# irconde/SSL4POLYP

Hardware: AMD Instinct MI355X
Metric: training-step images/sec/node, ViT-B/16 224^2 (cls fine-tune) (higher is better)
Workload: dtype bf16; 1 GPU; ViT-B/16 classification fine-tune, bs=64/GPU, 224^2, AdamW, random init, finetune mode full (finetune.py:49-91); global_batch=64, parallelism=dp1, launch=eager, lr_schedule=constant

## Files before the change

ssl4polyp_amd/csrc/pm_layernorm.hip:

```cpp
#include "pm_common.h"

namespace {

constexpr int kMaxD = 1280;

template <typename TOut, int NV>
__global__ __launch_bounds__(256) void ln_fwd_kernel(const float* __restrict__ x, long ldx, const float* __restrict__ gamma,
                                                     const float* __restrict__ beta, TOut* __restrict__ y,
                                                     float* __restrict__ mean_out, float* __restrict__ rstd_out, int M,
                                                     int D, float eps) {
  constexpr int kMaxVec = NV;
  const int lane = threadIdx.x & 63;
  const int wave = threadIdx.x >> 6;
  const int nvec = D >> 2;
  for (long row = (long)blockIdx.x * 4 + wave; row < M; row += (long)gridDim.x * 4) {
    const float* xr = x + row * ldx;
    f32x4 v[kMaxVec];
    float s = 0.f;
#pragma unroll
    for (int i = 0; i < kMaxVec; ++i) {
      const int c = lane + 64 * i;
      if (c < nvec) {
        v[i] = *reinterpret_cast<const f32x4*>(xr + 4 * c);
        s += (v[i][0] + v[i][1]) + (v[i][2] + v[i][3]);
// ... 31 lines not shown
      }
    }
  }
}

template <typename TDy, typename TAct, int NV>
__global__ __launch_bounds__(256) void ln_bwd_kernel(const TDy* __restrict__ dy, const float* __restrict__ x, long ldx,
                                                     const float* __restrict__ gamma, const float* __restrict__ mean,
                                                     const float* __restrict__ rstd, const float* __restrict__ dres,
                                                     long lddres, float* __restrict__ dx, long lddx,
                                                     TAct* __restrict__ dx_act, float* __restrict__ dgamma,
                                                     float* __restrict__ dbeta, float* __restrict__ dcolsum,
                                                     float* __restrict__ partials, int M, int D) {
  __shared__ float red[3][4][256 + 4];
  constexpr int kMaxVec = NV;
  const int lane = threadIdx.x & 63;
  const int wave = threadIdx.x >> 6;
  const int nvec = D >> 2;
  f32x4 g[kMaxVec];
  f32x4 acc_g[kMaxVec], acc_b[kMaxVec], acc_c[kMaxVec];
#pragma unroll
  for (int i = 0; i < kMaxVec; ++i) {
    const int c = lane + 64 * i;
    const f32x4 z = {0.f, 0.f, 0.f, 0.f};
    g[i] = (c < nvec) ? *reinterpret_cast<const f32x4*>(gamma + 4 * c) : z;
    acc_g[i] = z;
    acc_b[i] = z;
    acc_c[i] = z;
  }
  const float invD = 1.0f / (float)D;
  const long stride = (long)gridDim.x * 4;
  for (long row0 = (long)blockIdx.x * 4 + wave; row0 < M; row0 += 2 * stride) {
    long rows[2] = {row0, row0 + stride};
    const bool valid[2] = {true, rows[1] < M};
    if (!valid[1]) rows[1] = row0;
    float mu[2], rs[2], s1[2] = {0.f, 0.f}, s2[2] = {0.f, 0.f};
    f32x4 xh[2][kMaxVec], dv[2][kMaxVec], dr[2][kMaxVec];
#pragma unroll
    for (int u = 0; u < 2; ++u) {
      mu[u] = mean[rows[u]];
      rs[u] = rstd[rows[u]];
#pragma unroll
      for (int i = 0; i < kMaxVec; ++i) {
        const int c = lane + 64 * i;
        if (c < nvec) {
          xh[u][i] = *reinterpret_cast<const f32x4*>(x + rows[u] * ldx + 4 * c);
          dv[u][i] = load4<TDy>(dy + rows[u] * (long)D + 4 * c);
          if (dres) dr[u][i] = *reinterpret_cast<const f32x4*>(dres + rows[u] * lddres + 4 * c);
        }
      }
    }
#pragma unroll
    for (int u = 0; u < 2; ++u) {
      const float live = valid[u] ? 1.0f : 0.0f;
#pragma unroll
      for (int i = 0; i < kMaxVec; ++i) {
        const int c = lane + 64 * i;
        if (c < nvec) {
#pragma unroll
          for (int e = 0; e < 4; ++e) {
            xh[u][i][e] = (xh[u][i][e] - mu[u]) * rs[u];
            const float gg = dv[u][i][e] * g[i][e];
            s1[u] += gg;
            s2[u] += gg * xh[u][i][e];
            acc_g[i][e] += live * dv[u][i][e] * xh[u][i][e];
            acc_b[i][e] += live * dv[u][i][e];
          }
        }
      }
    }
    float c1[2], c2[2];
#pragma unroll
    for (int u = 0; u < 2; ++u) {
      c1[u] = s1[u];
      c2[u] = s2[u];
    }
#pragma unroll
    for (int o = 32; o > 0; o >>= 1) {
      c1[0] += __shfl_xor(c1[0], o, 64);
      c1[1] += __shfl_xor(c1[1], o, 64);
      c2[0] += __shfl_xor(c2[0], o, 64);
      c2[1] += __shfl_xor(c2[1], o, 64);
    }
#pragma unroll
    for (int u = 0; u < 2; ++u) {
      if (!valid[u]) continue;
      const float k1 = c1[u] * invD, k2 = c2[u] * invD;
#pragma unroll
      for (int i = 0; i < kMaxVec; ++i) {
        const int c = lane + 64 * i;
        if (c < nvec) {
          f32x4 o;
#pragma unroll
          for (int e = 0; e < 4; ++e) o[e] = rs[u] * (dv[u][i][e] * g[i][e] - k1 - xh[u][i][e] * k2);
          if (dres) o += dr[u][i];
          *reinterpret_cast<f32x4*>(dx + rows[u] * lddx + 4 * c) = o;
          if (dx_act) store4<TAct>(dx_act + rows[u] * (long)D + 4 * c, o);
#pragma unroll
          for (int e = 0; e < 4; ++e) acc_c[i][e] += o[e];
        }
      }
    }
  }
#pragma unroll
  for (int i = 0; i < kMaxVec; ++i) {
    const int c = lane + 64 * i;
    __syncthreads();
#pragma unroll
    for (int e = 0; e < 4; ++e) {
      red[0][wave][lane * 4 + e] = acc_g[i][e];
      red[1][wave][lane * 4 + e] = acc_b[i][e];
      red[2][wave][lane * 4 + e] = acc_c[i][e];
    }
    __syncthreads();
    if (wave < 3 && c < nvec) {
      float* dst = wave == 0 ? dgamma : (wave == 1 ? dbeta : dcolsum);
      if (dst) {
        f32x4 t;
#pragma unroll
        for (int e = 0; e < 4; ++e)
          t[e] = (red[wave][0][lane * 4 + e] + red[wave][1][lane * 4 + e]) +
                 (red[wave][2][lane * 4 + e] + red[wave][3][lane * 4 + e]);
        if (partials) {
          *reinterpret_cast<f32x4*>(partials + ((long)blockIdx.x * 3 + wave) * D + 4 * c) = t;
        } else {
#pragma unroll
          for (int e = 0; e < 4; ++e) atomicAdd(dst + 4 * c + e, t[e]);
        }
      }
    }
  }
}

__global__ __launch_bounds__(1024) void ln_bwd_reduce_kernel(const float* __restrict__ partials, float* dgamma, float* dbeta,
                                                             float* dcolsum, int nblocks, int D) {
  __shared__ float red[16][64];
  const int lane = threadIdx.x & 63, rg = threadIdx.x >> 6;
  const int d = blockIdx.x * 64 + lane;
  const int v = blockIdx.y;
  float* dst = v == 0 ? dgamma : (v == 1 ? dbeta : dcolsum);
  if (!dst) return;
  float s0 = 0.f;
  if (d < D) s0 = strided_sum<16>(partials + (long)v * D + d, 3L * D, rg, 16, nblocks);
  red[rg][lane] = s0;
  __syncthreads();
  if (rg == 0 && d < D) {
    float t = 0.f;
#pragma unroll
    for (int g = 0; g < 16; ++g) t += red[g][lane];
    dst[d] += t;
  }
}

inline int ln_grid(int M) {
  int g = (M + 3) / 4;
  return g < 1 ? 1 : (g > 1024 ? 1024 : g);
}

}

extern "C" int pm_layernorm_fwd(const float* x, long ldx, const float* gamma, const float* beta, void* y, int out_dtype,
                                float* mean, float* rstd, int M, int D, float eps, void* stream) {
  if (!x || !gamma || !beta || !y || !mean || !rstd) return PM_EINVAL;
  if (M <= 0 || D <= 0 || D > kMaxD || (D & 3) || (ldx & 3)) return PM_ESHAPE;
  const int grid = (M + 3) / 4 > 4096 ? 4096 : (M + 3) / 4;
#define PM_LN_FWD(TO, NV) \
  hipLaunchKernelGGL((ln_fwd_kernel<TO, NV>), dim3(grid), dim3(256), 0, pm_stream(stream), x, ldx, gamma, beta, (TO*)y, mean, rstd, M, D, eps)
  PM_DISPATCH_ACT(out_dtype, T, {
    if (D <= 1024) PM_LN_FWD(T, 4); else PM_LN_FWD(T, 5);
  });
#undef PM_LN_FWD
  return pm_check_launch();
}

extern "C" int pm_layernorm_bwd(const void* dy, int dy_dtype, const float* x, long ldx, const float* gamma,
                                const float* mean, const float* rstd, const float* dres, long lddres, float* dx,
                                long lddx, void* dx_act, int act_dtype, float* dgamma, float* dbeta, float* dcolsum,
                                int M, int D, void* workspace, size_t ws_bytes, void* stream) {
  if (!dy || !x || !gamma || !mean || !rstd || !dx) return PM_EINVAL;
  if (M <= 0 || D <= 0 || D > kMaxD || (D & 3) || (ldx & 3) || (lddx & 3) || (dres && (lddres & 3))) return PM_ESHAPE;
  if (dx_act && act_dtype != dy_dtype) return PM_EINVAL;
  int grid = (M + 3) / 4;
  float* partials = nullptr;
  const bool want_sums = dgamma || dbeta || dcolsum;
  if (want_sums && workspace && ws_bytes >= (size_t)64 * 3 * D * sizeof(float)) {
    int cap = (int)(ws_bytes / ((size_t)3 * D * sizeof(float)));
    if (cap > 1024) cap = 1024;
    if (grid > cap) grid = cap;
    partials = reinterpret_cast<float*>(workspace);
  } else if (grid > 256) {
    grid = 256;
  }
  if (grid < 1) grid = 1;
  hipStream_t s = pm_stream(stream);
  const int nv = (D + 255) / 256;
#define PM_LN_BWD(TD, NV)                                                                                               \
  hipLaunchKernelGGL((ln_bwd_kernel<TD, TD, NV>), dim3(grid), dim3(256), 0, s, (const TD*)dy, x, ldx, gamma, mean, rstd, \
                     dres, lddres, dx, lddx, (TD*)dx_act, dgamma, dbeta, dcolsum, partials, M, D)
  PM_DISPATCH_ACT(dy_dtype, T, {
    if (nv == 1) PM_LN_BWD(T, 1); else if (nv == 2) PM_LN_BWD(T, 2); else if (nv == 3) PM_LN_BWD(T, 3);
    else if (nv == 4) PM_LN_BWD(T, 4); else PM_LN_BWD(T, 5);
  });
#undef PM_LN_BWD
  if (partials)
    hipLaunchKernelGGL(ln_bwd_reduce_kernel, dim3((D + 63) / 64, 3), dim3(1024), 0, s, partials, dgamma, dbeta, dcolsum, grid, D);
  return pm_check_launch();
}
```

ssl4polyp_amd/csrc/pm_attention.hip:

```cpp
#include "pm_common.h"
#include <stdlib.h>

namespace {

template <int DH> constexpr int kTileUnroll = DH == 32 ? 2 : 1;

template <int RB> __device__ __forceinline__ int swz(int row) {
  if constexpr (RB == 64) return (row >> 2) & 3;
  else if constexpr (RB == 128) return (((row >> 1) & 1) << 2) | ((row >> 2) & 3);
  else if constexpr (RB == 384) return row & 7;
  else return row & 15;
}

template <typename T, int DH> constexpr int row_bytes() {
  return DH == 80 ? (sizeof(T) == 2 ? 256 : 384) : DH * (int)sizeof(T);
}

template <typename T, int DH>
__device__ __forceinline__ void load_image(char* img, const T* __restrict__ src, long ld, int rows_valid,
                                           int rows_total, int tid, int nthreads) {
  constexpr int RB = row_bytes<T, DH>();
  constexpr int CPV = DH * sizeof(T) / 16;
  constexpr int CPF = ((DH + 31) / 32) * 32 * sizeof(T) / 16;
  constexpr int EPC = 16 / sizeof(T);
  for (int id = tid; id < rows_total * CPF; id += nthreads) {
    const int row = id / CPF, c = id % CPF;
    u32x4 v = {0u, 0u, 0u, 0u};
    if (row < rows_valid && c < CPV) v = *reinterpret_cast<const u32x4*>(src + (long)row * ld + c * EPC);
    *reinterpret_cast<u32x4*>(img + row * RB + 16 * (c ^ swz<RB>(row))) = v;
  }
}

template <typename T, int DH>
__device__ __forceinline__ Frag16 frag_rows(const char* img, int rb, int kk, int lane) {
  constexpr int RB = row_bytes<T, DH>();
  const int row = rb + (lane & 31);
  const int c = 2 * kk + (lane >> 5);
  Frag16 f;
  f.u = *reinterpret_cast<const u32x4*>(img + row * RB + 16 * (c ^ swz<RB>(row)));
  return f;
}

template <typename T>
__device__ __forceinline__ Frag16 frag_global(const T* __restrict__ rowptr, bool valid, int kk, int lane) {
  constexpr int EPC = 16 / sizeof(T);
  Frag16 f;
  f.u = (u32x4){0u, 0u, 0u, 0u};
  if (valid) f.u = *reinterpret_cast<const u32x4*>(rowptr + (2 * kk + (lane >> 5)) * EPC);
  return f;
}

template <typename T, int DH>
__device__ __forceinline__ f32x16 mma_imgT_acc(const char* PM_LDS_IMAGE img, int rb, int d0, const f32x16& x, f32x16 acc, int lane) {
  constexpr int RB = row_bytes<T, DH>();
  if constexpr (sizeof(T) == 2) {
    const int g = lane >> 4, i = lane & 15, q = i >> 2, p = i & 3, hh = g >> 1;
    const int col = d0 + 16 * (g & 1) + 4 * p;
    const int c = col >> 3, sub = 8 * (p & 1);
    using lds_s4 = __attribute__((address_space(3))) short4v;
#pragma unroll
    for (int s = 0; s < 2; ++s) {
      Frag16 a, b;
      const int r0 = rb + 16 * s + 4 * hh + q;
      const int r1 = r0 + 8;
      const short4v lo = __builtin_amdgcn_ds_read_tr16_b64_v4i16((lds_s4*)(img + r0 * RB + 16 * (c ^ swz<RB>(r0)) + sub));
      const short4v hi = __builtin_amdgcn_ds_read_tr16_b64_v4i16((lds_s4*)(img + r1 * RB + 16 * (c ^ swz<RB>(r1)) + sub));
      a.u[0] = ((unsigned)(unsigned short)lo[0]) | (((unsigned)(unsigned short)lo[1]) << 16);
      a.u[1] = ((unsigned)(unsigned short)lo[2]) | (((unsigned)(unsigned short)lo[3]) << 16);
      a.u[2] = ((unsigned)(unsigned short)hi[0]) | (((unsigned)(unsigned short)hi[1]) << 16);
      a.u[3] = ((unsigned)(unsigned short)hi[2]) | (((unsigned)(unsigned short)hi[3]) << 16);
#pragma unroll
      for (int j = 0; j < 8; ++j) frag_set<T>(b, j, x[8 * s + j]);
      acc = mfma16B<T>(a, b, acc);
    }
  } else {
    const int hh = lane >> 5;
    const int col = d0 + (lane & 31);
#pragma unroll
    for (int r = 0; r < 16; ++r) {
      const int row = rb + acc_row(r, hh);
      const float a = *reinterpret_cast<const float*>(img + row * RB + 16 * ((col >> 2) ^ swz<RB>(row)) + 4 * (col & 3));
      acc = __builtin_amdgcn_mfma_f32_32x32x2f32(a, x[r], acc, 0, 0, 0);
    }
  }
  return acc;
}

__device__ __forceinline__ f32x16 zero16() {
  f32x16 z;
#pragma unroll
  for (int r = 0; r < 16; ++r) z[r] = 0.f;
  return z;
}

template <typename T>
__device__ __forceinline__ void store_tile_T(T* __restrict__ rowptr, bool valid, const f32x16& acc, float scale, int lane,
                                             int ncols = 32) {
  if (!valid) return;
  const int hh = lane >> 5;
#pragma unroll
  for (int g = 0; g < 4; ++g) {
    f32x4 v = {acc[4 * g] * scale, acc[4 * g + 1] * scale, acc[4 * g + 2] * scale, acc[4 * g + 3] * scale};
    if (8 * g + 4 * hh < ncols) store4<T>(rowptr + 8 * g + 4 * hh, v);
  }
}
template <int DH> __device__ __forceinline__ constexpr int tile_cols(int dt) { return DH - 32 * dt < 32 ? DH - 32 * dt : 32; }

constexpr float kLog2e = 1.4426950408889634f;

struct QkvLayout {
  long ld, which_stride, head_stride, batch_stride;
};
inline QkvLayout qkv_layout(int B, int N, int H, int DH, bool head_major) {
  if (head_major) return QkvLayout{(long)DH, (long)B * H * N * DH, (long)N * DH, (long)H * N * DH};
  return QkvLayout{3L * H * DH, (long)H * DH, (long)DH, (long)N * 3L * H * DH};
}
inline bool attn_head_major() {
  static const bool v = [] { const char* e = getenv("PM_ATTN_HEADMAJOR"); return e && e[0] == '1'; }();
  return v;
}

template <int DH> __device__ __forceinline__ int problem_of_block(int bid, int nprob, int H) {
  if constexpr (DH == 32) {
#ifndef PM_ATTN_NO_PAIR_MAP
    if ((nprob & 15) == 0 && (H & 1) == 0) {
      const int xcd = bid & 7, j = bid >> 3;
      return (((j >> 1) << 3) + xcd) * 2 + (j & 1);
    }
#endif
  }
  return bid;
}

template <int NT> struct Waves { static constexpr int value = NT; };

template <typename T, int DH, int NT> constexpr int chunk_tiles() {
  constexpr int per_tile = 2 * 32 * row_bytes<T, DH>() + 2 * 32 * (int)sizeof(float);
  if (NT * per_tile <= 150 * 1024) return NT;
  return (80 * 1024) / per_tile;
}

template <typename T, int DH, int NT, int CT>
__global__ __launch_bounds__(Waves<NT>::value * 64) void attn_fwd_kernel(const T* __restrict__ qkv, T* __restrict__ out,
                                                                        float* __restrict__ lse, int N, int H,
                                                                        float scale) {
  constexpr int RB = row_bytes<T, DH>();
  constexpr int KS = DH * sizeof(T) / 32;
  constexpr int DT = (DH + 31) / 32;
  constexpr int NW = Waves<NT>::value;
  static_assert(NW == NT, "one wave per query tile: its softmax state stays in registers across key chunks");
  extern __shared__ __attribute__((aligned(16))) char smem[];
  char* imgK = smem;
  char* imgV = smem + CT * 32 * RB;
  const int tid = threadIdx.x, lane = tid & 63, wave = tid >> 6, hh = lane >> 5;
  const int prob = problem_of_block<DH>(blockIdx.x, gridDim.x, H);
  const int b = prob / H, h = prob % H;
  const long ld = 3L * H * DH;
  const T* base = qkv + (long)b * N * ld + h * DH;
  const float c = scale * kLog2e;
  const int q = wave * 32 + (lane & 31);
  const bool qv = q < N;
  Frag16 fq[KS];
  f32x16 o[DT];
#pragma unroll
  for (int dt = 0; dt < DT; ++dt) o[dt] = zero16();
  float m = -INFINITY, l = 0.f;
  for (int c0 = 0; c0 < NT; c0 += CT) {
    if (c0) __syncthreads();
    load_image<T, DH>(imgK, base + H * DH + (long)c0 * 32 * ld, ld, N - c0 * 32, CT * 32, tid, NW * 64);
    load_image<T, DH>(imgV, base + 2 * H * DH + (long)c0 * 32 * ld, ld, N - c0 * 32, CT * 32, tid, NW * 64);
    __syncthreads();
    if (c0 == 0) {
#pragma unroll
      for (int kk = 0; kk < KS; ++kk) fq[kk] = frag_global<T>(base + (long)q * ld, qv, kk, lane);
    }
    const int cend = c0 + CT < NT ? c0 + CT : NT;
#pragma unroll 1
    for (int kt = c0; kt < cend; ++kt) {
      const int rb = (kt - c0) * 32;
      f32x16 s = zero16();
#pragma unroll
      for (int kk = 0; kk < KS; ++kk) s = mfma16B<T>(frag_rows<T, DH>(imgK, rb, kk, lane), fq[kk], s);
      float tm = -INFINITY;
      if (kt * 32 + 32 > N) {
#pragma unroll
        for (int r = 0; r < 16; ++r) {
          const int key = kt * 32 + acc_row(r, hh);
          s[r] = key < N ? s[r] : -INFINITY;
        }
      }
#pragma unroll
      for (int r = 0; r < 16; ++r) tm = fmaxf(tm, s[r]);
      tm = fmaxf(tm, __shfl_xor(tm, 32, 64));
      const float mn = fmaxf(m, tm);
      const float alpha = __builtin_amdgcn_exp2f((m - mn) * c);
      const float mnc = mn * c;
      float ts = 0.f;
#pragma unroll
      for (int r = 0; r < 16; ++r) {
        s[r] = __builtin_amdgcn_exp2f(s[r] * c - mnc);
        ts += s[r];
      }
      l = l * alpha + ts;
      const bool moved = __builtin_amdgcn_ballot_w64(mn != m) != 0;
      m = mn;
#pragma unroll
      for (int dt = 0; dt < DT; ++dt) {
        if (moved) {
#pragma unroll
          for (int r = 0; r < 16; ++r) o[dt][r] *= alpha;
        }
        o[dt] = mma_imgT_acc<T, DH>(imgV, rb, dt * 32, s, o[dt], lane);
      }
    }
  }
  l += __shfl_xor(l, 32, 64);
  if (qv && hh == 0) lse[((long)b * H + h) * N + q] = m * scale + __logf(l);
  const float inv = 1.0f / l;
  T* orow = out + ((long)b * N + q) * H * DH + h * DH;
#pragma unroll
  for (int dt = 0; dt < DT; ++dt) store_tile_T<T>(orow + dt * 32, qv, o[dt], inv, lane, tile_cols<DH>(dt));
}

// ... 316 lines not shown
  const int b = prob / H, h = prob % H;
  const long ld = 3L * H * DH, ldo = (long)H * DH;
  const T* base = qkv + (long)b * lay.batch_stride + (long)h * lay.head_stride;
  const T* dobase = dout + (long)b * N * ldo + h * DH;
#pragma unroll
  for (int i = 0; i < (PCS + NT - 1) / NT; ++i) {
    const int p = wave + NT * i;
    if (p < PCS) {
      dma_rows<RB>(imgQ, base, lay.ld, N, p, lane);
      dma_rows<RB>(imgK, base + lay.which_stride, lay.ld, N, p, lane);
      dma_rows<RB>(imgV, base + 2 * lay.which_stride, lay.ld, N, p, lane);
      dma_rows<RB>(imgDO, dobase, ldo, N, p, lane);
    }
  }
  const int q = wave * 32 + (lane & 31);
  const bool qv = q < N;
  const long sidx = ((long)b * H + h) * N;
  Frag16 fo[KS];
  {
    const T* orow = out + ((long)b * N + (qv ? q : N - 1)) * ldo + h * DH;
#pragma unroll
    for (int kk = 0; kk < KS; ++kk) fo[kk].u = *reinterpret_cast<const u32x4*>(orow + (2 * kk + hh) * 8);
  }
  for (int i = tid; i < NT * 32; i += NT * 64) sl2[i] = i < N ? lse[sidx + i] * kLog2e : 0.f;
  asm volatile("s_waitcnt vmcnt(0)" ::: "memory");
  __syncthreads();
  {
    const int pad0 = N, npad = NT * 32 - N;
    for (int i = tid; i < npad * CPR; i += NT * 64) {
      const int off = (pad0 + i / CPR) * RB + 16 * (i % CPR);
      const u32x4 z = {0u, 0u, 0u, 0u};
      *reinterpret_cast<u32x4*>(imgQ + off) = z;
      *reinterpret_cast<u32x4*>(imgK + off) = z;
      *reinterpret_cast<u32x4*>(imgV + off) = z;
      *reinterpret_cast<u32x4*>(imgDO + off) = z;
    }
  }
  __syncthreads();
  const float c = scale * kLog2e;
  Frag16 fq[KS], fdo[KS];
  float dl = 0.f;
#pragma unroll
  for (int kk = 0; kk < KS; ++kk) {
    fq[kk] = frag_rows<T, DH>(imgQ, wave * 32, kk, lane);
    fdo[kk] = frag_rows<T, DH>(imgDO, wave * 32, kk, lane);
#pragma unroll
    for (int e = 0; e < 8; ++e) dl += frag_get<T>(fdo[kk], e) * frag_get<T>(fo[kk], e);
  }
  dl += __shfl_xor(dl, 32, 64);
  if (!qv) dl = 0.f;
  if (hh == 0) sdl[q] = dl * scale;
  {
    const float l2 = sl2[q];
    const float dls = dl * scale;
    f32x16 dq[DT];
#pragma unroll
    for (int dt = 0; dt < DT; ++dt) dq[dt] = zero16();
#pragma unroll kTileUnroll<DH>
    for (int kt = 0; kt < ((dbg & 1) ? 0 : NT); ++kt) {
      f32x16 s = zero16(), dp = zero16();
#pragma unroll
      for (int kk = 0; kk < KS; ++kk) {
        s = mfma16B<T>(frag_rows<T, DH>(imgK, kt * 32, kk, lane), fq[kk], s);
        dp = mfma16B<T>(frag_rows<T, DH>(imgV, kt * 32, kk, lane), fdo[kk], dp);
      }
#pragma unroll
      for (int r = 0; r < 16; ++r) s[r] = __builtin_amdgcn_exp2f(fminf(s[r] * c - l2, 0.f)) * (dp[r] * scale - dls);
#pragma unroll
      for (int dt = 0; dt < DT; ++dt) dq[dt] = mma_imgT_acc<T, DH>(imgK, kt * 32, dt * 32, s, dq[dt], lane);
    }
    T* dqrow = dqkv + ((long)b * N + q) * ld + h * DH;
#pragma unroll
    for (int dt = 0; dt < DT; ++dt) store_tile_T<T>(dqrow + dt * 32, qv, dq[dt], 1.0f, lane);
  }
  __syncthreads();
  {
    const int key = q;
    const bool kv = qv;
    Frag16 fk[KS], fv[KS];
#pragma unroll
    for (int kk = 0; kk < KS; ++kk) {
      fk[kk] = frag_rows<T, DH>(imgK, wave * 32, kk, lane);
      fv[kk] = frag_rows<T, DH>(imgV, wave * 32, kk, lane);
    }
    f32x16 dk[DT], dv[DT];
#pragma unroll
    for (int dt = 0; dt < DT; ++dt) {
      dk[dt] = zero16();
      dv[dt] = zero16();
    }
#pragma unroll kTileUnroll<DH>
    for (int qt = 0; qt < ((dbg & 2) ? 0 : NT); ++qt) {
      f32x16 s = zero16(), dp = zero16();
#pragma unroll
      for (int kk = 0; kk < KS; ++kk) {
        s = mfma16B<T>(frag_rows<T, DH>(imgQ, qt * 32, kk, lane), fk[kk], s);
        dp = mfma16B<T>(frag_rows<T, DH>(imgDO, qt * 32, kk, lane), fv[kk], dp);
      }
#pragma unroll
      for (int g = 0; g < 4; ++g) {
        const int qq = qt * 32 + 8 * g + 4 * hh;
        const f32x4 l4 = *reinterpret_cast<const f32x4*>(sl2 + qq);
        const f32x4 d4 = *reinterpret_cast<const f32x4*>(sdl + qq);
#pragma unroll
        for (int e = 0; e < 4; ++e) {
          const int r = 4 * g + e;
          const float pr = __builtin_amdgcn_exp2f(fminf(s[r] * c - l4[e], 0.f));
          s[r] = pr;
          dp[r] = pr * (dp[r] * scale - d4[e]);
        }
      }
#pragma unroll
      for (int dt = 0; dt < DT; ++dt) {
        dv[dt] = mma_imgT_acc<T, DH>(imgDO, qt * 32, dt * 32, s, dv[dt], lane);
        dk[dt] = mma_imgT_acc<T, DH>(imgQ, qt * 32, dt * 32, dp, dk[dt], lane);
      }
    }
    T* drow = dqkv + ((long)b * N + key) * ld + h * DH;
#pragma unroll
    for (int dt = 0; dt < DT; ++dt) {
      store_tile_T<T>(drow + H * DH + dt * 32, kv, dk[dt], 1.0f, lane);
      store_tile_T<T>(drow + 2 * H * DH + dt * 32, kv, dv[dt], 1.0f, lane);
    }
  }
}

template <typename T, int DH, int NT>
int launch_bwd_fused(const void* qkv, const void* out, const void* dout, const float* lse, void* dqkv, int B, int N, int H,
                     hipStream_t s) {
  const size_t lds = 4 * NT * 32 * DH * 2 + 2 * NT * 32 * sizeof(float);
  const float scale = 1.0f / sqrtf((float)DH);
  auto kern = attn_bwd_fused_kernel<T, DH, NT>;
  PM_ALLOW_LDS(kern, lds);
#ifdef PM_ATTN_DEBUG
  static const int dbg = [] { const char* e = getenv("PM_ATTN_BWD_SKIP"); return e ? atoi(e) : 0; }();
  hipLaunchKernelGGL(kern, dim3(B * H), dim3(NT * 64), lds, s, (const T*)qkv, (const T*)out, (const T*)dout, lse,
                     (T*)dqkv, N, H, scale, qkv_layout(B, N, H, DH, attn_head_major()), dbg);
#else
  hipLaunchKernelGGL(kern, dim3(B * H), dim3(NT * 64), lds, s, (const T*)qkv, (const T*)out, (const T*)dout, lse,
                     (T*)dqkv, N, H, scale, qkv_layout(B, N, H, DH, attn_head_major()));
#endif
  return pm_check_launch();
}

template <typename T, int DH>
int dispatch_bwd_fused(int nt, const void* qkv, const void* out, const void* dout, const float* lse, void* dqkv, int B, int N,
                       int H, hipStream_t s) {
  if (nt <= 1) return launch_bwd_fused<T, DH, 1>(qkv, out, dout, lse, dqkv, B, N, H, s);
  if (nt <= 2) return launch_bwd_fused<T, DH, 2>(qkv, out, dout, lse, dqkv, B, N, H, s);
  if (nt <= 7) return launch_bwd_fused<T, DH, 7>(qkv, out, dout, lse, dqkv, B, N, H, s);
  return launch_bwd_fused<T, DH, 9>(qkv, out, dout, lse, dqkv, B, N, H, s);
}

template <typename T, int DH, int NT>
int launch_bwd(const void* qkv, const void* out, const void* dout, const float* lse, float* delta, void* dqkv, int B,
               int N, int H, hipStream_t s) {
  constexpr int NW = Waves<NT>::value;
  constexpr int CT = chunk_tiles<T, DH, NT>();
  const size_t lds = 2 * CT * 32 * row_bytes<T, DH>();
  const size_t lds_kv = lds + 2 * CT * 32 * sizeof(float);
  const float scale = 1.0f / sqrtf((float)DH);
  auto kq = attn_bwd_q_kernel<T, DH, NT, CT>;
  auto kkv = attn_bwd_kv_kernel<T, DH, NT, CT>;
  PM_ALLOW_LDS(kq, lds);
  PM_ALLOW_LDS(kkv, lds_kv);
  hipLaunchKernelGGL(kq, dim3(B * H), dim3(NW * 64), lds, s, (const T*)qkv, (const T*)out, (const T*)dout, lse, delta,
                     (T*)dqkv, N, H, scale);
  hipLaunchKernelGGL(kkv, dim3(B * H), dim3(NW * 64), lds_kv, s, (const T*)qkv, (const T*)dout, lse,
                     (const float*)delta, (T*)dqkv, N, H, scale);
  return pm_check_launch();
}

template <typename T, int DH>
int dispatch_fwd(int nt, const void* qkv, void* out, float* lse, int B, int N, int H, hipStream_t s) {
  if constexpr (DH == 80) {
    if (nt <= 3) return launch_fwd<T, DH, 3>(qkv, out, lse, B, N, H, s);
    return launch_fwd<T, DH, 9>(qkv, out, lse, B, N, H, s);
  } else {
    if (nt <= 1) return launch_fwd<T, DH, 1>(qkv, out, lse, B, N, H, s);
    if (nt <= 2) return launch_fwd<T, DH, 2>(qkv, out, lse, B, N, H, s);
    if (nt <= 7) return launch_fwd<T, DH, 7>(qkv, out, lse, B, N, H, s);
    return launch_fwd<T, DH, 9>(qkv, out, lse, B, N, H, s);
  }
}
template <typename T, int DH>
int dispatch_bwd(int nt, const void* qkv, const void* out, const void* dout, const float* lse, float* delta, void* dqkv,
                 int B, int N, int H, hipStream_t s) {
  if constexpr (DH == 80) {
    if (nt <= 3) return launch_bwd<T, DH, 3>(qkv, out, dout, lse, delta, dqkv, B, N, H, s);
    return launch_bwd<T, DH, 9>(qkv, out, dout, lse, delta, dqkv, B, N, H, s);
  } else {
    if (nt <= 1) return launch_bwd<T, DH, 1>(qkv, out, dout, lse, delta, dqkv, B, N, H, s);
    if (nt <= 2) return launch_bwd<T, DH, 2>(qkv, out, dout, lse, delta, dqkv, B, N, H, s);
    if (nt <= 7) return launch_bwd<T, DH, 7>(qkv, out, dout, lse, delta, dqkv, B, N, H, s);
    return launch_bwd<T, DH, 9>(qkv, out, dout, lse, delta, dqkv, B, N, H, s);
  }
}

bool attn_v1() {
  static const bool v = [] { const char* e = getenv("PM_ATTN_V1"); return e && e[0] == '1'; }();
  return v;
}
bool attn_fwd2_dh32() {
  static const bool v = [] { const char* e = getenv("PM_ATTN_FWD2_DH32"); return e && e[0] == '1'; }();
  return v;
}

inline int check_shape(int B, int N, int H, int dh, int dtype) {
  if (B <= 0 || N <= 0 || H <= 0) return PM_ESHAPE;
  if (N > 288) return PM_ESHAPE;
  if (dh != 32 && dh != 64 && dh != 80) return PM_ESHAPE;
  if (dtype != PM_BF16 && dtype != PM_F16 && dtype != PM_F32) return PM_EINVAL;
  return PM_OK;
}

}

extern "C" int pm_attention_fwd(const void* qkv, void* out, float* lse, int B, int N, int H, int dh, int dtype,
                                void* stream) {
  if (!qkv || !out || !lse) return PM_EINVAL;
  const int st = check_shape(B, N, H, dh, dtype);
  if (st) return st;
  const int nt = (N + 31) / 32;
  hipStream_t s = pm_stream(stream);
  if (dtype != PM_F32) {
    PM_DISPATCH_16(dtype, T, {
      if (nt == 7 && dh == 64 && !attn_v1()) return launch_fwd2<T, 64>(qkv, out, lse, B, N, H, s);
      if (nt == 7 && dh == 32 && attn_fwd2_dh32()) return launch_fwd2<T, 32>(qkv, out, lse, B, N, H, s);
      if (dh == 80) return dispatch_fwd<T, 80>(nt, qkv, out, lse, B, N, H, s);
      return dh == 64 ? dispatch_fwd<T, 64>(nt, qkv, out, lse, B, N, H, s) : dispatch_fwd<T, 32>(nt, qkv, out, lse, B, N, H, s);
    });
  }
  if (dh == 80) return dispatch_fwd<float, 80>(nt, qkv, out, lse, B, N, H, s);
  return dh == 64 ? dispatch_fwd<float, 64>(nt, qkv, out, lse, B, N, H, s)
                  : dispatch_fwd<float, 32>(nt, qkv, out, lse, B, N, H, s);
}

extern "C" int pm_attention_bwd(const void* qkv, const void* out, const void* dout, const float* lse, float* delta,
                                void* dqkv, int B, int N, int H, int dh, int dtype, void* stream) {
  if (!qkv || !out || !dout || !lse || !delta || !dqkv) return PM_EINVAL;
  const int st = check_shape(B, N, H, dh, dtype);
  if (st) return st;
  const int nt = (N + 31) / 32;
  hipStream_t s = pm_stream(stream);
  if (dtype != PM_F32) {
    PM_DISPATCH_16(dtype, T, {
      if (dh == 80) return dispatch_bwd<T, 80>(nt, qkv, out, dout, lse, delta, dqkv, B, N, H, s);
      if (!attn_v1())
        return dh == 64 ? dispatch_bwd_fused<T, 64>(nt, qkv, out, dout, lse, dqkv, B, N, H, s)
                        : dispatch_bwd_fused<T, 32>(nt, qkv, out, dout, lse, dqkv, B, N, H, s);
      return dh == 64 ? dispatch_bwd<T, 64>(nt, qkv, out, dout, lse, delta, dqkv, B, N, H, s)
                      : dispatch_bwd<T, 32>(nt, qkv, out, dout, lse, delta, dqkv, B, N, H, s);
    });
  }
  if (dh == 80) return dispatch_bwd<float, 80>(nt, qkv, out, dout, lse, delta, dqkv, B, N, H, s);
  return dh == 64 ? dispatch_bwd<float, 64>(nt, qkv, out, dout, lse, delta, dqkv, B, N, H, s)
                  : dispatch_bwd<float, 32>(nt, qkv, out, dout, lse, delta, dqkv, B, N, H, s);
}
```

Baseline: 6264 images/sec.

## Add software-prefetching LayerNorm forward/backward kernels with persistent grid

Adds new LayerNorm forward and backward kernels that prefetch the next row's inputs into registers while the current row is computed. Each block now loops over several rows or virtual blocks, and the grids are capped by env-tunable defaults (1024 forward, 256 backward). The aim is to hide global-memory latency with fewer, longer-lived blocks. The cost is higher register pressure and possibly lower occupancy. The old kernels stay reachable through PM_LN_LEGACY.

```diff
diff --git a/ssl4polyp_amd/csrc/pm_layernorm.hip b/ssl4polyp_amd/csrc/pm_layernorm.hip
--- a/ssl4polyp_amd/csrc/pm_layernorm.hip
+++ b/ssl4polyp_amd/csrc/pm_layernorm.hip
@@ -207,9 +207,255 @@
   }
 }
 
-inline int ln_grid(int M) {
-  int g = (M + 3) / 4;
-  return g < 1 ? 1 : (g > 1024 ? 1024 : g);
+template <typename T> using Raw4 = T __attribute__((ext_vector_type(4)));
+template <typename T> __device__ __forceinline__ Raw4<T> load_raw4(const T* p) { return *reinterpret_cast<const Raw4<T>*>(p); }
+template <typename T> __device__ __forceinline__ f32x4 widen4(Raw4<T> v) {
+  if constexpr (sizeof(T) == 4) return v;
+  else return f32x4{(float)v[0], (float)v[1], (float)v[2], (float)v[3]};
+}
+
+template <typename TOut, int NV>
+__global__ __launch_bounds__(256) void ln_fwd_pipe_kernel(const float* __restrict__ x, long ldx, const float* __restrict__ gamma,
+                                                          const float* __restrict__ beta, TOut* __restrict__ y,
+                                                          float* __restrict__ mean_out, float* __restrict__ rstd_out, int M,
+                                                          int D, float eps) {
+  const int lane = threadIdx.x & 63;
+  const int wave = threadIdx.x >> 6;
+  const int nvec = D >> 2;
+  const long stride = (long)gridDim.x * 4;
+  long row = (long)blockIdx.x * 4 + wave;
+  f32x4 nx[NV];
+  if (row < M) {
+#pragma unroll
+    for (int i = 0; i < NV; ++i)
+      if (lane + 64 * i < nvec) nx[i] = *reinterpret_cast<const f32x4*>(x + row * ldx + 4 * (lane + 64 * i));
+  }
+  for (; row < M; row += stride) {
+    f32x4 v[NV];
+#pragma unroll
+    for (int i = 0; i < NV; ++i) v[i] = nx[i];
+    const long nrow = row + stride;
+    if (nrow < M) {
+#pragma unroll
+      for (int i = 0; i < NV; ++i)
+        if (lane + 64 * i < nvec) nx[i] = *reinterpret_cast<const f32x4*>(x + nrow * ldx + 4 * (lane + 64 * i));
+    }
+    float s = 0.f;
+#pragma unroll
+    for (int i = 0; i < NV; ++i)
+      if (lane + 64 * i < nvec) s += (v[i][0] + v[i][1]) + (v[i][2] + v[i][3]);
+    const float mean = wave_sum(s) / (float)D;
+    float q = 0.f;
+#pragma unroll
+    for (int i = 0; i < NV; ++i) {
+      if (lane + 64 * i < nvec) {
+#pragma unroll
+        for (int e = 0; e < 4; ++e) {
+          const float d = v[i][e] - mean;
+          q += d * d;
+        }
+      }
+    }
+    const float rstd = rsqrtf(wave_sum(q) / (float)D + eps);
+    if (lane == 0) {
+      mean_out[row] = mean;
+      rstd_out[row] = rstd;
+    }
+    TOut* yr = y + row * (long)D;
+#pragma unroll
+    for (int i = 0; i < NV; ++i) {
+      const int c = lane + 64 * i;
+      if (c < nvec) {
+        const f32x4 g = *reinterpret_cast<const f32x4*>(gamma + 4 * c);
+        const f32x4 b = *reinterpret_cast<const f32x4*>(beta + 4 * c);
+        f32x4 o;
+#pragma unroll
+        for (int e = 0; e < 4; ++e) o[e] = (v[i][e] - mean) * rstd * g[e] + b[e];
+        store4<TOut>(yr + 4 * c, o);
+      }
+    }
+  }
+}
+
+template <typename TDy, typename TAct, int NV>
+__global__ __launch_bounds__(256) void ln_bwd_pipe_kernel(const TDy* __restrict__ dy, const float* __restrict__ x, long ldx,
+                                                          const float* __restrict__ gamma, const float* __restrict__ mean,
+                                                          const float* __restrict__ rstd, const float* __restrict__ dres,
+                                                          long lddres, float* __restrict__ dx, long lddx,
+                                                          TAct* __restrict__ dx_act, float* __restrict__ dgamma,
+                                                          float* __restrict__ dbeta, float* __restrict__ dcolsum,
+                                                          float* __restrict__ partials, int M, int D, int nvb) {
+  __shared__ float red[3][4][256 + 4];
+  const int lane = threadIdx.x & 63;
+  const int wave = threadIdx.x >> 6;
+  const int nvec = D >> 2;
+  const bool want_sums = dgamma || dbeta || dcolsum;
+  f32x4 g[NV];
+#pragma unroll
+  for (int i = 0; i < NV; ++i) {
+    const int c = lane + 64 * i;
+    const f32x4 z = {0.f, 0.f, 0.f, 0.f};
+    g[i] = (c < nvec) ? *reinterpret_cast<const f32x4*>(gamma + 4 * c) : z;
+  }
+  const float invD = 1.0f / (float)D;
+  const long stride = (long)nvb * 4;
+  f32x4 px[NV], pr[NV];
+  Raw4<TDy> pd[NV];
+  float pmu = 0.f, prs = 0.f;
+  auto prefetch = [&](long r) {
+    pmu = mean[r];
+    prs = rstd[r];
+#pragma unroll
+    for (int i = 0; i < NV; ++i) {
+      const int c = lane + 64 * i;
+      if (c < nvec) {
+        px[i] = *reinterpret_cast<const f32x4*>(x + r * ldx + 4 * c);
+        pd[i] = load_raw4<TDy>(dy + r * (long)D + 4 * c);
+        if (dres) pr[i] = *reinterpret_cast<const f32x4*>(dres + r * lddres + 4 * c);
+      }
+    }
+  };
+  if ((long)blockIdx.x * 4 + wave < M) prefetch((long)blockIdx.x * 4 + wave);
+  for (int vb = blockIdx.x; vb < nvb; vb += gridDim.x) {
+    f32x4 acc_g[NV], acc_b[NV], acc_c[NV];
+#pragma unroll
+    for (int i = 0; i < NV; ++i) {
+      const f32x4 z = {0.f, 0.f, 0.f, 0.f};
+      acc_g[i] = z;
+      acc_b[i] = z;
+      acc_c[i] = z;
+    }
+    for (long row = (long)vb * 4 + wave; row < M; row += stride) {
+      const float mu = pmu, rs = prs;
+      f32x4 xh[NV], dr[NV];
+      Raw4<TDy> dd[NV];
+#pragma unroll
+      for (int i = 0; i < NV; ++i) {
+        xh[i] = px[i];
+        dd[i] = pd[i];
+        dr[i] = pr[i];
+      }
+      long nrow = row + stride;
+      if (nrow >= M) nrow = vb + (int)gridDim.x < nvb ? ((long)vb + gridDim.x) * 4 + wave : M;
+      if (nrow < M) prefetch(nrow);
+      float s1 = 0.f, s2 = 0.f;
+      f32x4 dv[NV];
+#pragma unroll
+      for (int i = 0; i < NV; ++i) {
+        const int c = lane + 64 * i;
+        if (c < nvec) {
+          dv[i] = widen4<TDy>(dd[i]);
+#pragma unroll
+          for (int e = 0; e < 4; ++e) {
+            xh[i][e] = (xh[i][e] - mu) * rs;
+            const float gg = dv[i][e] * g[i][e];
+            s1 += gg;
+            s2 += gg * xh[i][e];
+            acc_g[i][e] += dv[i][e] * xh[i][e];
+            acc_b[i][e] += dv[i][e];
+          }
+        }
+      }
+#pragma unroll
+      for (int o = 32; o > 0; o >>= 1) {
+        s1 += __shfl_xor(s1, o, 64);
+        s2 += __shfl_xor(s2, o, 64);
+      }
+      const float k1 = s1 * invD, k2 = s2 * invD;
+#pragma unroll
+      for (int i = 0; i < NV; ++i) {
+        const int c = lane + 64 * i;
+        if (c < nvec) {
+          f32x4 o;
+#pragma unroll
+          for (int e = 0; e < 4; ++e) o[e] = rs * (dv[i][e] * g[i][e] - k1 - xh[i][e] * k2);
+          if (dres) o += dr[i];
+          *reinterpret_cast<f32x4*>(dx + row * lddx + 4 * c) = o;
+          if (dx_act) store4<TAct>(dx_act + row * (long)D + 4 * c, o);
+#pragma unroll
+          for (int e = 0; e < 4; ++e) acc_c[i][e] += o[e];
+        }
+      }
+    }
+    if (!want_sums) continue;
+#pragma unroll
+    for (int i = 0; i < NV; ++i) {
+      const int c = lane + 64 * i;
+      __syncthreads();
+#pragma unroll
+      for (int e = 0; e < 4; ++e) {
+        red[0][wave][lane * 4 + e] = acc_g[i][e];
+        red[1][wave][lane * 4 + e] = acc_b[i][e];
+        red[2][wave][lane * 4 + e] = acc_c[i][e];
+      }
+      __syncthreads();
+      if (wave < 3 && c < nvec) {
+        f32x4 t;
+#pragma unroll
+        for (int e = 0; e < 4; ++e)
+          t[e] = (red[wave][0][lane * 4 + e] + red[wave][1][lane * 4 + e]) + (red[wave][2][lane * 4 + e] + red[wave][3][lane * 4 + e]);
+        if (partials) {
+          *reinterpret_cast<f32x4*>(partials + ((long)vb * 3 + wave) * D + 4 * c) = t;
+        } else {
+          float* dst = wave == 0 ? dgamma : (wave == 1 ? dbeta : dcolsum);
+          if (dst) {
+#pragma unroll
+            for (int e = 0; e < 4; ++e) atomicAdd(dst + 4 * c + e, t[e]);
+          }
+        }
+      }
+    }
+  }
+}
+
+inline bool ln_legacy() {
+  static const bool v = [] { const char* e = getenv("PM_LN_LEGACY"); return e && e[0] == '1'; }();
+  return v;
+}
+inline int ln_fwd_blocks() {
+  static const int v = [] { const char* e = getenv("PM_LN_FWD_BLOCKS"); return e && e[0] ? atoi(e) : 1024; }();
+  return v < 1 ? 1 : v;
+}
+inline int ln_bwd_blocks() {
+  static const int v = [] { const char* e = getenv("PM_LN_BWD_BLOCKS"); return e && e[0] ? atoi(e) : 256; }();
+  return v < 1 ? 1 : (v > 1024 ? 1024 : v);
+}
+
+inline int ln_bwd_legacy_grid(int M, int D, bool want_sums, void* workspace, size_t ws_bytes, float** partials) {
+  int grid = (M + 3) / 4;
+  *partials = nullptr;
+  if (want_sums && workspace && ws_bytes >= (size_t)64 * 3 * D * sizeof(float)) {
+    int cap = (int)(ws_bytes / ((size_t)3 * D * sizeof(float)));
+    if (cap > 1024) cap = 1024;
+    if (grid > cap) grid = cap;
+    *partials = reinterpret_cast<float*>(workspace);
+  } else if (grid > 256) {
+    grid = 256;
+  }
+  return grid < 1 ? 1 : grid;
+}
+
+int ln_bwd_pipe(const void* dy, int dy_dtype, const float* x, long ldx, const float* gamma, const float* mean, const float* rstd,
+                const float* dres, long lddres, float* dx, long lddx, void* dx_act, float* dgamma, float* dbeta, float* dcolsum,
+                int M, int D, void* workspace, size_t ws_bytes, hipStream_t s) {
+  float* partials = nullptr;
+  const int nvb = ln_bwd_legacy_grid(M, D, dgamma || dbeta || dcolsum, workspace, ws_bytes, &partials);
+  int grid = (M + 15) / 16;
+  if (grid > ln_bwd_blocks()) grid = ln_bwd_blocks();
+  if (grid > nvb) grid = nvb;
+  if (grid < 1) grid = 1;
+  const int nv = (D + 255) / 256;
+#define PM_LN_BWD(TD, NV)                                                                                                    \
+  hipLaunchKernelGGL((ln_bwd_pipe_kernel<TD, TD, NV>), dim3(grid), dim3(256), 0, s, (const TD*)dy, x, ldx, gamma, mean, rstd, \
+                     dres, lddres, dx, lddx, (TD*)dx_act, dgamma, dbeta, dcolsum, partials, M, D, nvb)
+  PM_DISPATCH_ACT(dy_dtype, T, {
+    if (nv == 1) PM_LN_BWD(T, 1); else if (nv == 2) PM_LN_BWD(T, 2); else if (nv == 3) PM_LN_BWD(T, 3);
+    else if (nv == 4) PM_LN_BWD(T, 4); else PM_LN_BWD(T, 5);
+  });
+#undef PM_LN_BWD
+  if (partials)
+    hipLaunchKernelGGL(ln_bwd_reduce_kernel, dim3((D + 63) / 64, 3), dim3(1024), 0, s, partials, dgamma, dbeta, dcolsum, nvb, D);
+  return pm_check_launch();
 }
 
 }
@@ -218,11 +464,24 @@
                                 float* mean, float* rstd, int M, int D, float eps, void* stream) {
   if (!x || !gamma || !beta || !y || !mean || !rstd) return PM_EINVAL;
   if (M <= 0 || D <= 0 || D > kMaxD || (D & 3) || (ldx & 3)) return PM_ESHAPE;
-  const int grid = (M + 3) / 4 > 4096 ? 4096 : (M + 3) / 4;
+  if (ln_legacy()) {
+    const int grid = (M + 3) / 4 > 4096 ? 4096 : (M + 3) / 4;
 #define PM_LN_FWD(TO, NV) \
   hipLaunchKernelGGL((ln_fwd_kernel<TO, NV>), dim3(grid), dim3(256), 0, pm_stream(stream), x, ldx, gamma, beta, (TO*)y, mean, rstd, M, D, eps)
+    PM_DISPATCH_ACT(out_dtype, T, {
+      if (D <= 1024) PM_LN_FWD(T, 4); else PM_LN_FWD(T, 5);
+    });
+#undef PM_LN_FWD
+    return pm_check_launch();
+  }
+  int grid = (M + 7) / 8;
+  if (grid > ln_fwd_blocks()) grid = ln_fwd_blocks();
+  const int nv = (D + 255) / 256;
+#define PM_LN_FWD(TO, NV) \
+  hipLaunchKernelGGL((ln_fwd_pipe_kernel<TO, NV>), dim3(grid), dim3(256), 0, pm_stream(stream), x, ldx, gamma, beta, (TO*)y, mean, rstd, M, D, eps)
   PM_DISPATCH_ACT(out_dtype, T, {
-    if (D <= 1024) PM_LN_FWD(T, 4); else PM_LN_FWD(T, 5);
+    if (nv == 1) PM_LN_FWD(T, 1); else if (nv == 2) PM_LN_FWD(T, 2); else if (nv == 3) PM_LN_FWD(T, 3);
+    else if (nv == 4) PM_LN_FWD(T, 4); else PM_LN_FWD(T, 5);
   });
 #undef PM_LN_FWD
   return pm_check_launch();
@@ -235,18 +494,10 @@
   if (!dy || !x || !gamma || !mean || !rstd || !dx) return PM_EINVAL;
   if (M <= 0 || D <= 0 || D > kMaxD || (D & 3) || (ldx & 3) || (lddx & 3) || (dres && (lddres & 3))) return PM_ESHAPE;
   if (dx_act && act_dtype != dy_dtype) return PM_EINVAL;
-  int grid = (M + 3) / 4;
+  if (!ln_legacy()) return ln_bwd_pipe(dy, dy_dtype, x, ldx, gamma, mean, rstd, dres, lddres, dx, lddx, dx_act, dgamma, dbeta,
+                                       dcolsum, M, D, workspace, ws_bytes, pm_stream(stream));
   float* partials = nullptr;
-  const bool want_sums = dgamma || dbeta || dcolsum;
-  if (want_sums && workspace && ws_bytes >= (size_t)64 * 3 * D * sizeof(float)) {
-    int cap = (int)(ws_bytes / ((size_t)3 * D * sizeof(float)));
-    if (cap > 1024) cap = 1024;
-    if (grid > cap) grid = cap;
-    partials = reinterpret_cast<float*>(workspace);
-  } else if (grid > 256) {
-    grid = 256;
-  }
-  if (grid < 1) grid = 1;
+  const int grid = ln_bwd_legacy_grid(M, D, dgamma || dbeta || dcolsum, workspace, ws_bytes, &partials);
   hipStream_t s = pm_stream(stream);
   const int nv = (D + 255) / 256;
 #define PM_LN_BWD(TD, NV)                                                                                               \
```

Result: no change. 6232 images/sec (median of 2 runs) (-0.5%).

## Add single-pass attention backward kernel that stores dS in LDS and reuses it for dQ

Applied to the files above, without the earlier changes.

Adds a new bf16/fp16 attention backward kernel for head dim 64 and 7 tiles (N=197, i.e. ViT-B/16) that computes P and dS once per key tile. It stores dS in LDS, then reuses that buffer for the dQ pass instead of recomputing QK^T and dP. K and V are staged in the dS region, and the K image is rewritten over Q after the dK/dV phase. This is meant to remove the duplicated score and softmax recomputation of the existing fused backward. The cost is a large LDS footprint (about 150KB per block), which limits occupancy, plus an env flag to fall back to the old path.

```diff
diff --git a/ssl4polyp_amd/csrc/pm_attention.hip b/ssl4polyp_amd/csrc/pm_attention.hip
--- a/ssl4polyp_amd/csrc/pm_attention.hip
+++ b/ssl4polyp_amd/csrc/pm_attention.hip
@@ -50,25 +50,32 @@
   return f;
 }
 
+template <int RB>
+__device__ __forceinline__ Frag16 frag_tr(const char* PM_LDS_IMAGE img, int rb, int s, int col0, int lane) {
+  const int g = lane >> 4, i = lane & 15, q = i >> 2, p = i & 3, hh = g >> 1;
+  const int col = col0 + 16 * (g & 1) + 4 * p;
+  const int c = col >> 3, sub = 8 * (p & 1);
+  using lds_s4 = __attribute__((address_space(3))) short4v;
+  const int r0 = rb + 16 * s + 4 * hh + q;
+  const int r1 = r0 + 8;
+  const short4v lo = __builtin_amdgcn_ds_read_tr16_b64_v4i16((lds_s4*)(img + r0 * RB + 16 * (c ^ swz<RB>(r0)) + sub));
+  const short4v hi = __builtin_amdgcn_ds_read_tr16_b64_v4i16((lds_s4*)(img + r1 * RB + 16 * (c ^ swz<RB>(r1)) + sub));
+  Frag16 a;
+  a.u[0] = ((unsigned)(unsigned short)lo[0]) | (((unsigned)(unsigned short)lo[1]) << 16);
+  a.u[1] = ((unsigned)(unsigned short)lo[2]) | (((unsigned)(unsigned short)lo[3]) << 16);
+  a.u[2] = ((unsigned)(unsigned short)hi[0]) | (((unsigned)(unsigned short)hi[1]) << 16);
+  a.u[3] = ((unsigned)(unsigned short)hi[2]) | (((unsigned)(unsigned short)hi[3]) << 16);
+  return a;
+}
+
 template <typename T, int DH>
 __device__ __forceinline__ f32x16 mma_imgT_acc(const char* PM_LDS_IMAGE img, int rb, int d0, const f32x16& x, f32x16 acc, int lane) {
   constexpr int RB = row_bytes<T, DH>();
   if constexpr (sizeof(T) == 2) {
-    const int g = lane >> 4, i = lane & 15, q = i >> 2, p = i & 3, hh = g >> 1;
-    const int col = d0 + 16 * (g & 1) + 4 * p;
-    const int c = col >> 3, sub = 8 * (p & 1);
-    using lds_s4 = __attribute__((address_space(3))) short4v;
 #pragma unroll
     for (int s = 0; s < 2; ++s) {
-      Frag16 a, b;
-      const int r0 = rb + 16 * s + 4 * hh + q;
-      const int r1 = r0 + 8;
-      const short4v lo = __builtin_amdgcn_ds_read_tr16_b64_v4i16((lds_s4*)(img + r0 * RB + 16 * (c ^ swz<RB>(r0)) + sub));
-      const short4v hi = __builtin_amdgcn_ds_read_tr16_b64_v4i16((lds_s4*)(img + r1 * RB + 16 * (c ^ swz<RB>(r1)) + sub));
-      a.u[0] = ((unsigned)(unsigned short)lo[0]) | (((unsigned)(unsigned short)lo[1]) << 16);
-      a.u[1] = ((unsigned)(unsigned short)lo[2]) | (((unsigned)(unsigned short)lo[3]) << 16);
-      a.u[2] = ((unsigned)(unsigned short)hi[0]) | (((unsigned)(unsigned short)hi[1]) << 16);
-      a.u[3] = ((unsigned)(unsigned short)hi[2]) | (((unsigned)(unsigned short)hi[3]) << 16);
+      const Frag16 a = frag_tr<RB>(img, rb, s, d0, lane);
+      Frag16 b;
 #pragma unroll
       for (int j = 0; j < 8; ++j) frag_set<T>(b, j, x[8 * s + j]);
       acc = mfma16B<T>(a, b, acc);
@@ -691,6 +698,179 @@
   return launch_bwd_fused<T, DH, 9>(qkv, out, dout, lse, dqkv, B, N, H, s);
 }
 
+template <typename T, int DH, int NT> struct BwdOnceLds {
+  static constexpr int IMG = NT * 32 * DH * 2;
+  static constexpr int DSB = NT * 32 * 64;
+  static constexpr int bytes = 2 * IMG + NT * DSB + 2 * NT * 32 * (int)sizeof(float);
+  static_assert(2 * IMG <= NT * DSB, "the K and V images are staged in the dS region");
+  static_assert(bytes <= 160 * 1024, "LDS of one CU");
+};
+
+template <typename T, int DH, int NT>
+__global__ __launch_bounds__(NT * 64) void attn_bwd_once_kernel(const T* __restrict__ qkv, const T* __restrict__ out,
+                                                               const T* __restrict__ dout, const float* __restrict__ lse,
+                                                               T* __restrict__ dqkv, int N, int H, float scale, QkvLayout lay) {
+  static_assert(sizeof(T) == 2, "16-bit operands");
+  using L = BwdOnceLds<T, DH, NT>;
+  constexpr int RB = DH * 2;
+  constexpr int IMG = L::IMG;
+  constexpr int DSB = L::DSB;
+  constexpr int PCS = IMG / 1024;
+  constexpr int KS = RB / 32;
+  constexpr int DT = DH / 32;
+  constexpr int CPR = RB / 16;
+  extern __shared__ __attribute__((aligned(16))) char smem[];
+  char* imgQ = smem;
+  char* imgDO = smem + IMG;
+  char* imgDS = smem + 2 * IMG;
+  char* imgK = imgDS;
+  char* imgV = imgDS + IMG;
+  char* imgKB = smem;
+  float* sl2 = reinterpret_cast<float*>(smem + 2 * IMG + NT * DSB);
+  float* sdl = sl2 + NT * 32;
+  const int tid = threadIdx.x, lane = tid & 63, hh = lane >> 5;
+  const int wave = __builtin_amdgcn_readfirstlane(tid >> 6);
+  const int prob = problem_of_block<DH>(blockIdx.x, gridDim.x, H);
+  const int b = prob / H, h = prob % H;
+  const long ld = 3L * H * DH, ldo = (long)H * DH;
+  const T* base = qkv + (long)b * lay.batch_stride + (long)h * lay.head_stride;
+  const T* dobase = dout + (long)b * N * ldo + h * DH;
+#pragma unroll
+  for (int i = 0; i < (PCS + NT - 1) / NT; ++i) {
+    const int p = wave + NT * i;
+    if (p < PCS) {
+      dma_rows<RB>(imgQ, base, lay.ld, N, p, lane);
+      dma_rows<RB>(imgK, base + lay.which_stride, lay.ld, N, p, lane);
+      dma_rows<RB>(imgV, base + 2 * lay.which_stride, lay.ld, N, p, lane);
+      dma_rows<RB>(imgDO, dobase, ldo, N, p, lane);
+    }
+  }
+  const int q = wave * 32 + (lane & 31);
+  const bool qv = q < N;
+  const long sidx = ((long)b * H + h) * N;
+  Frag16 fo[KS];
+  {
+    const T* orow = out + ((long)b * N + (qv ? q : N - 1)) * ldo + h * DH;
+#pragma unroll
+    for (int kk = 0; kk < KS; ++kk) fo[kk].u = *reinterpret_cast<const u32x4*>(orow + (2 * kk + hh) * 8);
+  }
+  for (int i = tid; i < NT * 32; i += NT * 64) sl2[i] = i < N ? lse[sidx + i] * kLog2e : 0.f;
+  asm volatile("s_waitcnt vmcnt(0)" ::: "memory");
+  __syncthreads();
+  {
+    const int pad0 = N, npad = NT * 32 - N;
+    for (int i = tid; i < npad * CPR; i += NT * 64) {
+      const int off = (pad0 + i / CPR) * RB + 16 * (i % CPR);
+      const u32x4 z = {0u, 0u, 0u, 0u};
+      *reinterpret_cast<u32x4*>(imgQ + off) = z;
+      *reinterpret_cast<u32x4*>(imgK + off) = z;
+      *reinterpret_cast<u32x4*>(imgV + off) = z;
+      *reinterpret_cast<u32x4*>(imgDO + off) = z;
+    }
+  }
+  __syncthreads();
+  const float c = scale * kLog2e;
+  float dl = 0.f;
+  Frag16 fk[KS], fv[KS];
+#pragma unroll
+  for (int kk = 0; kk < KS; ++kk) {
+    const Frag16 fdo = frag_rows<T, DH>(imgDO, wave * 32, kk, lane);
+#pragma unroll
+    for (int e = 0; e < 8; ++e) dl += frag_get<T>(fdo, e) * frag_get<T>(fo[kk], e);
+    fk[kk] = frag_rows<T, DH>(imgK, wave * 32, kk, lane);
+    fv[kk] = frag_rows<T, DH>(imgV, wave * 32, kk, lane);
+  }
+  dl += __shfl_xor(dl, 32, 64);
+  if (!qv) dl = 0.f;
+  if (hh == 0) sdl[q] = dl * scale;
+  asm volatile("s_waitcnt lgkmcnt(0)" ::: "memory");
+  __builtin_amdgcn_sched_barrier(0);
+  __syncthreads();
+  {
+    const int krow = wave * 32 + (lane & 31);
+    f32x16 dk[DT], dv[DT];
+#pragma unroll
+    for (int dt = 0; dt < DT; ++dt) {
+      dk[dt] = zero16();
+      dv[dt] = zero16();
+    }
+#pragma unroll 1
+    for (int qt = 0; qt < NT; ++qt) {
+      f32x16 s = zero16(), dp = zero16();
+#pragma unroll
+      for (int kk = 0; kk < KS; ++kk) {
+        s = mfma16B<T>(frag_rows<T, DH>(imgQ, qt * 32, kk, lane), fk[kk], s);
+        dp = mfma16B<T>(frag_rows<T, DH>(imgDO, qt * 32, kk, lane), fv[kk], dp);
+      }
+      char* blk = imgDS + qt * DSB + krow * 64;
+#pragma unroll
+      for (int g = 0; g < 4; ++g) {
+        const int qq = qt * 32 + 8 * g + 4 * hh;
+        const f32x4 l4 = *reinterpret_cast<const f32x4*>(sl2 + qq);
+        const f32x4 d4 = *reinterpret_cast<const f32x4*>(sdl + qq);
+        Frag16 w;
+#pragma unroll
+        for (int e = 0; e < 4; ++e) {
+          const int r = 4 * g + e;
+          const float pr = __builtin_amdgcn_exp2f(fminf(s[r] * c - l4[e], 0.f));
+          s[r] = pr;
+          dp[r] = pr * (dp[r] * scale - d4[e]);
+          frag_set<T>(w, e, dp[r]);
+        }
+        *reinterpret_cast<u32x2*>(blk + 16 * (g ^ swz<64>(krow)) + 8 * hh) = (u32x2){w.u[0], w.u[1]};
+      }
+#pragma unroll
+      for (int dt = 0; dt < DT; ++dt) {
+        dv[dt] = mma_imgT_acc<T, DH>(imgDO, qt * 32, dt * 32, s, dv[dt], lane);
+        dk[dt] = mma_imgT_acc<T, DH>(imgQ, qt * 32, dt * 32, dp, dk[dt], lane);
+      }
+    }
+    T* drow = dqkv + ((long)b * N + q) * ld + h * DH;
+#pragma unroll
+    for (int dt = 0; dt < DT; ++dt) {
+      store_tile_T<T>(drow + H * DH + dt * 32, qv, dk[dt], 1.0f, lane);
+      store_tile_T<T>(drow + 2 * H * DH + dt * 32, qv, dv[dt], 1.0f, lane);
+    }
+  }
+  __syncthreads();
+#pragma unroll
+  for (int kk = 0; kk < KS; ++kk) {
+    const int row = wave * 32 + (lane & 31), ch = 2 * kk + hh;
+    *reinterpret_cast<u32x4*>(imgKB + row * RB + 16 * (ch ^ swz<RB>(row))) = fk[kk].u;
+  }
+  __syncthreads();
+  {
+    const char* blk = imgDS + wave * DSB;
+    f32x16 dq[DT];
+#pragma unroll
+    for (int dt = 0; dt < DT; ++dt) dq[dt] = zero16();
+#pragma unroll 1
+    for (int kt = 0; kt < NT; ++kt) {
+      const Frag16 b0 = frag_tr<64>(blk, kt * 32, 0, 0, lane), b1 = frag_tr<64>(blk, kt * 32, 1, 0, lane);
+#pragma unroll
+      for (int dt = 0; dt < DT; ++dt) {
+        dq[dt] = mfma16B<T>(frag_tr<RB>(imgKB, kt * 32, 0, dt * 32, lane), b0, dq[dt]);
+        dq[dt] = mfma16B<T>(frag_tr<RB>(imgKB, kt * 32, 1, dt * 32, lane), b1, dq[dt]);
+      }
+    }
+    T* dqrow = dqkv + ((long)b * N + q) * ld + h * DH;
+#pragma unroll
+    for (int dt = 0; dt < DT; ++dt) store_tile_T<T>(dqrow + dt * 32, qv, dq[dt], 1.0f, lane);
+  }
+}
+
+template <typename T, int DH, int NT>
+int launch_bwd_once(const void* qkv, const void* out, const void* dout, const float* lse, void* dqkv, int B, int N, int H,
+                    hipStream_t s) {
+  constexpr size_t lds = BwdOnceLds<T, DH, NT>::bytes;
+  const float scale = 1.0f / sqrtf((float)DH);
+  auto kern = attn_bwd_once_kernel<T, DH, NT>;
+  PM_ALLOW_LDS(kern, lds);
+  hipLaunchKernelGGL(kern, dim3(B * H), dim3(NT * 64), lds, s, (const T*)qkv, (const T*)out, (const T*)dout, lse, (T*)dqkv,
+                     N, H, scale, qkv_layout(B, N, H, DH, attn_head_major()));
+  return pm_check_launch();
+}
+
 template <typename T, int DH, int NT>
 int launch_bwd(const void* qkv, const void* out, const void* dout, const float* lse, float* delta, void* dqkv, int B,
                int N, int H, hipStream_t s) {
@@ -740,6 +920,10 @@
   static const bool v = [] { const char* e = getenv("PM_ATTN_V1"); return e && e[0] == '1'; }();
   return v;
 }
+bool attn_bwd_twice() {
+  static const bool v = [] { const char* e = getenv("PM_ATTN_BWD_TWICE"); return e && e[0] == '1'; }();
+  return v;
+}
 bool attn_fwd2_dh32() {
   static const bool v = [] { const char* e = getenv("PM_ATTN_FWD2_DH32"); return e && e[0] == '1'; }();
   return v;
@@ -785,6 +969,8 @@
   if (dtype != PM_F32) {
     PM_DISPATCH_16(dtype, T, {
       if (dh == 80) return dispatch_bwd<T, 80>(nt, qkv, out, dout, lse, delta, dqkv, B, N, H, s);
+      if (!attn_v1() && dh == 64 && nt == 7 && !attn_bwd_twice())
+        return launch_bwd_once<T, 64, 7>(qkv, out, dout, lse, dqkv, B, N, H, s);
       if (!attn_v1())
         return dh == 64 ? dispatch_bwd_fused<T, 64>(nt, qkv, out, dout, lse, dqkv, B, N, H, s)
                         : dispatch_bwd_fused<T, 32>(nt, qkv, out, dout, lse, dqkv, B, N, H, s);
```

Result: no change. 6375 images/sec before, 6415 images/sec after (median of 6 runs) (+0.6%).
